# thecasterian/fluca

Hardware: AMD Instinct MI355X
Metric: pressure-Poisson Jacobi-PCG iterations/s, 512^3 cells per GPU (higher is better)
Workload: dtype f64

## Files before the change

### fluca_amd/csrc/fl_knobs.h

```cpp
#pragma once
#include <atomic>

#define FL_PUBLIC_KNOBS(X)                                                                                                                   \
  X(cheb_fuse, 1)                   \
  X(placement, 0)                           \
  X(cg_xbatch, 1)                                           \
  X(cg_xdepth, 8)                 \
  X(cheb_zero3, 1)                  \
  X(mg_prolong, 1)                                                             \
  X(mg_flexible, 1)                                                             \
  X(mg_coarse, 1)                                   \
  X(mg_post_smooth, 0)               \
  X(schur_var_fused, 1)      \
  X(overlap, 1)              \
  X(comm_loopback, 0)           \
  X(comm_trace, 0)                             \
  X(ghost_width, 0)                                       \
  X(placement_verbose, 0)                                                                        \
  X(placement_vmm, 1)                    \
  X(allreduce, 0)

namespace fl {

enum Knob : int {
#define X(n, d) K_##n,
  FL_PUBLIC_KNOBS(X)
#undef X
      K_COUNT
};

int         knob(Knob k);
void        knob_set(Knob k, int v);
int         knob_find(const char *name);
const char *knob_name(int k);

}
```

### fluca_amd/csrc/fl_mg.hip

```cpp
#include <new>

#include "fl_handle.h"
#include "fl_device.h"

namespace fl {

struct Owned {
  int64_t npair_row, npairs;
};
__device__ __forceinline__ Owned owned_of(const GridP &g)
{
  Owned o;
  o.npair_row = (g.nx + 1) / 2;
  o.npairs    = o.npair_row * (int64_t)g.ny * g.nz;
  return o;
}
__device__ __forceinline__ int64_t pair_off(const GridP &g, const Owned &o, int64_t q, bool &two)
{
  const int     ip = (int)(q % o.npair_row);
  const int64_t row = q / o.npair_row;
  const int     j = (int)(row % g.ny), k = (int)(row / g.ny);
  two = 2 * ip + 1 < g.nx;
  return g.off0 + (int64_t)k * g.sxy + (int64_t)j * g.sx + 2 * ip;
}
__device__ __forceinline__ double2 ldp(const double *a, int64_t off, bool two) { return two ? *reinterpret_cast<const double2 *>(a + off) : make_double2(a[off], 0.); }
__device__ __forceinline__ void    stp(double *a, int64_t off, bool two, double2 v)
{
  if (two) *reinterpret_cast<double2 *>(a + off) = v;
  else a[off] = v.x;
}

__global__ void __launch_bounds__(256) k_mg_restrict(GridP gc, GridP gf, int rx, int ry, int rz, const double *__restrict__ wx, const double *__restrict__ wy, const double *__restrict__ wz,
                                                     const double *__restrict__ fine, double *__restrict__ coarse)
{
  const int64_t n = (int64_t)gc.nx * gc.ny * gc.nz;
  for (int64_t q = (int64_t)blockIdx.x * blockDim.x + threadIdx.x; q < n; q += (int64_t)gridDim.x * blockDim.x) {
    const int     I = (int)(q % gc.nx);
    const int64_t t = q / gc.nx;
    const int     J = (int)(t % gc.ny), K = (int)(t / gc.ny);
    double        s = 0.;
    for (int c = 0; c < rz; ++c)
      for (int b = 0; b < ry; ++b) {
        const int     j = J * ry + b, k = K * rz + c;
        const int64_t ro = gf.off0 + (int64_t)k * gf.sxy + (int64_t)j * gf.sx + (int64_t)I * rx;
        const double  wyz = wy[j] * wz[k];
        if (rx == 2) {
          const double2 f = *reinterpret_cast<const double2 *>(fine + ro);
          s += wyz * (wx[2 * I] * f.x + wx[2 * I + 1] * f.y);
        } else s += wyz * wx[I] * fine[ro];
      }
    coarse[gc.off0 + (int64_t)K * gc.sxy + (int64_t)J * gc.sx + I] = s;
  }
}

__global__ void __launch_bounds__(256) k_mg_prolong_add(GridP gf, GridP gc, int rx, int ry, int rz, const double *__restrict__ coarse, double *__restrict__ fine)
{
  const Owned o = owned_of(gf);
  for (int64_t q = (int64_t)blockIdx.x * blockDim.x + threadIdx.x; q < o.npairs; q += (int64_t)gridDim.x * blockDim.x) {
    const int     ip = (int)(q % o.npair_row);
    const int64_t row = q / o.npair_row;
    const int     j = (int)(row % gf.ny), k = (int)(row / gf.ny), i = 2 * ip;
    const bool    two = i + 1 < gf.nx;
    const int64_t fo = gf.off0 + (int64_t)k * gf.sxy + (int64_t)j * gf.sx + i;
    const int64_t co = gc.off0 + (int64_t)(k / rz) * gc.sxy + (int64_t)(j / ry) * gc.sx;
    double2       f = ldp(fine, fo, two);
    f.x += coarse[co + i / rx];
    if (two) f.y += coarse[co + (i + 1) / rx];
    stp(fine, fo, two, f);
  }
}

struct MgLin {
  const int    *pn[3];
  const double *pw[3];
};

__global__ void __launch_bounds__(256) k_mg_prolong_lin_tile(GridP gf, GridP gc, int rx, int ry, int rz, MgLin t, const double *__restrict__ coarse, double *__restrict__ fine, int zc)
{
  const int lane = threadIdx.x & 63, w = __builtin_amdgcn_readfirstlane(threadIdx.x >> 6);
  const int i = ((int)blockIdx.x * 64 + lane) * 2, j = (int)blockIdx.y * 4 + w;
  if (j >= gf.ny || i >= gf.nx) return;
  const int     k0 = (int)blockIdx.z * zc, k1 = min(k0 + zc, gf.nz);
  const bool    two = i + 1 < gf.nx;
  const int     i1 = two ? i + 1 : i;
  const int     I0 = i / rx, I1 = i1 / rx, J = j / ry;
  const int     ox0 = t.pn[0][i], ox1 = t.pn[0][i1];
  const double  wx0 = t.pw[0][i], wx1 = t.pw[0][i1];
  const double  wy = t.pw[1][j];
  const int64_t oy = (int64_t)t.pn[1][j] * gc.sx;
  const double *cj = coarse + gc.off0 + (int64_t)J * gc.sx;
  double       *fj = fine + gf.off0 + (int64_t)j * gf.sx + i;
  for (int k = k0; k < k1; ++k) {
    const int     K = k / rz;
    const double  wz = t.pw[2][k];
    const int64_t oz = (int64_t)t.pn[2][k] * gc.sxy;
    const double *ck = cj + (int64_t)K * gc.sxy;
    double        v0[4], v1[4];
#pragma unroll
    for (int a = 0; a < 4; ++a) {
      const double *line = ck + ((a & 1) ? oy : 0) + ((a & 2) ? oz : 0);
      const double  p0 = line[I0], p1 = line[I1];
      v0[a] = fma(wx0, line[I0 + ox0] - p0, p0);
      v1[a] = fma(wx1, line[I1 + ox1] - p1, p1);
    }
    const double a0 = fma(wy, v0[1] - v0[0], v0[0]), b0 = fma(wy, v0[3] - v0[2], v0[2]);
    const double a1 = fma(wy, v1[1] - v1[0], v1[0]), b1 = fma(wy, v1[3] - v1[2], v1[2]);
    const int64_t fo = (int64_t)k * gf.sxy;
    double2       f = ldp(fj, fo, two);
    f.x += fma(wz, b0 - a0, a0);
    if (two) f.y += fma(wz, b1 - a1, a1);
    stp(fj, fo, two, f);
  }
}

template <int CTRL>
__device__ __forceinline__ double mg_lane_shift(double v)
{
  const int lo = __builtin_amdgcn_update_dpp(__double2loint(v), __double2loint(v), CTRL, 0xf, 0xf, false);
  const int hi = __builtin_amdgcn_update_dpp(__double2hiint(v), __double2hiint(v), CTRL, 0xf, 0xf, false);
  return __hiloint2double(hi, lo);
}
__global__ void __launch_bounds__(256) k_mg_prolong_lin_cc(GridP gf, GridP gc, MgLin t, const double *__restrict__ coarse, double *__restrict__ fine, int kc)
{
  const int lane = threadIdx.x & 63, w = __builtin_amdgcn_readfirstlane(threadIdx.x >> 6);
  const int J = (int)blockIdx.y * 4 + w;
  if (J >= gc.ny) return;
  const int  I = (int)blockIdx.x * 62 - 1 + lane, Ic = min(I, gc.nx);
  const bool act = lane >= 1 && lane <= 62 && I < gc.nx;
  const int  K0 = (int)blockIdx.z * kc, K1 = min(K0 + kc, gc.nz);
  const int  ia = act ? 2 * I : 0;
  const int    ox[2] = {t.pn[0][ia], t.pn[0][ia + 1]};
  const double wx[2] = {t.pw[0][ia], t.pw[0][ia + 1]};
  const int    oy[2] = {t.pn[1][2 * J], t.pn[1][2 * J + 1]};
  const double wy[2] = {t.pw[1][2 * J], t.pw[1][2 * J + 1]};
  const double *cb = coarse + gc.off0 + (int64_t)J * gc.sx + Ic;
  auto plane = [&](int K, double (&X)[3][2]) {
    const double *cp = cb + (int64_t)K * gc.sxy;
#pragma unroll
    for (int jj = 0; jj < 3; ++jj) {
      const double C = cp[(int64_t)(jj - 1) * gc.sx];
      const double L = mg_lane_shift<0x138>(C), R = mg_lane_shift<0x130>(C);
#pragma unroll
      for (int a = 0; a < 2; ++a) {
        const double N = ox[a] < 0 ? L : (ox[a] > 0 ? R : C);
        X[jj][a] = fma(wx[a], N - C, C);
      }
    }
  };
  double Xm[3][2], Xc[3][2], Xp[3][2];
  plane(K0 - 1, Xm);
  plane(K0, Xc);
  for (int K = K0; K < K1; ++K) {
    plane(K + 1, Xp);
#pragma unroll
    for (int c = 0; c < 2; ++c) {
      const int    k = 2 * K + c, oz = t.pn[2][k];
      const double wz = t.pw[2][k];
#pragma unroll
      for (int b = 0; b < 2; ++b) {
        double2 add;
#pragma unroll
        for (int a = 0; a < 2; ++a) {
          const double v0 = Xc[1][a], v1 = oy[b] < 0 ? Xc[0][a] : (oy[b] > 0 ? Xc[2][a] : Xc[1][a]);
          const double z0 = oz < 0 ? Xm[1][a] : (oz > 0 ? Xp[1][a] : Xc[1][a]);
          const double z1 = oz < 0 ? (oy[b] < 0 ? Xm[0][a] : (oy[b] > 0 ? Xm[2][a] : Xm[1][a]))
                                   : (oz > 0 ? (oy[b] < 0 ? Xp[0][a] : (oy[b] > 0 ? Xp[2][a] : Xp[1][a])) : v1);
          const double A = fma(wy[b], v1 - v0, v0), B = fma(wy[b], z1 - z0, z0);
          (a ? add.y : add.x) = fma(wz, B - A, A);
        }
        if (act) {
          double2 *f = reinterpret_cast<double2 *>(fine + gf.off0 + (int64_t)k * gf.sxy + (int64_t)(2 * J + b) * gf.sx + 2 * I);
          double2  v = *f;
          v.x += add.x;
          v.y += add.y;
          *f = v;
        }
      }
    }
#pragma unroll
    for (int jj = 0; jj < 3; ++jj)
#pragma unroll
      for (int a = 0; a < 2; ++a) {
        Xm[jj][a] = Xc[jj][a];
        Xc[jj][a] = Xp[jj][a];
      }
  }
}

__global__ void __launch_bounds__(256) k_mg_dots(GridP g, const double *__restrict__ z, const double *__restrict__ r, double *__restrict__ partial, int stride)
{
  __shared__ double red[5 * 4];
  double            v[5] = {0., 0., 0., 0., 0.};
  const Owned       o = owned_of(g);
  for (int64_t q = (int64_t)blockIdx.x * blockDim.x + threadIdx.x; q < o.npairs; q += (int64_t)gridDim.x * blockDim.x) {
    bool          two;
    const int64_t off = pair_off(g, o, q, two);
    const double2 zv = ldp(z, off, two), rv = ldp(r, off, two);
    v[0] += zv.x + zv.y;
    v[1] += zv.x * zv.x + zv.y * zv.y;
    v[2] += rv.x * zv.x + rv.y * zv.y;
    v[3] += rv.x + rv.y;
    v[4] += rv.x * rv.x + rv.y * rv.y;
  }
  block_sum<5>(v, red);
  if (threadIdx.x == 0)
#pragma unroll
    for (int a = 0; a < 5; ++a) partial[(int64_t)a * stride + blockIdx.x] = v[a];
}

template <int OP>
__global__ void __launch_bounds__(256) k_mg_pw(GridP g, double a, double b, double c, const double *__restrict__ x0, const double *__restrict__ x1, double *__restrict__ y0, double *__restrict__ y1)
{
  const int     lane = threadIdx.x & 63, w = __builtin_amdgcn_readfirstlane(threadIdx.x >> 6), nw = blockDim.x >> 6;
  const int     nseg = (g.nx + 127) / 128;
  const int64_t nitem = (int64_t)nseg * g.ny * g.nz;
  for (int64_t it = (int64_t)blockIdx.x * nw + w; it < nitem; it += (int64_t)gridDim.x * nw) {
    const int seg = (int)(it % nseg), row = (int)(it / nseg);
    const int j = row % g.ny, k = row / g.ny, i = seg * 128 + 2 * lane;
    if (i >= g.nx) continue;
    const bool    two = i + 1 < g.nx;
    const int64_t off = g.off0 + (int64_t)k * g.sxy + (int64_t)j * g.sx + i;
    if (OP == 0) {
      const double2 xv = ldp(x0, off, two), yv = ldp(y0, off, two);
      stp(y0, off, two, make_double2((xv.x - c) + b * yv.x, (xv.y - c) + b * yv.y));
    } else if (OP == 1) {
      const double2 pv = ldp(x0, off, two), qv = ldp(x1, off, two), xv = ldp(y0, off, two), rv = ldp(y1, off, two);
      stp(y0, off, two, make_double2(xv.x + a * pv.x, xv.y + a * pv.y));
      stp(y1, off, two, make_double2(rv.x - a * qv.x, rv.y - a * qv.y));
    } else if (OP == 3) {
      const double2 pv = ldp(x0, off, two), xv = ldp(y0, off, two);
      stp(y0, off, two, make_double2(xv.x + a * pv.x, xv.y + a * pv.y));
    } else if (OP == 4) {
      const double2 zv = ldp(x0, off, two), pv = ldp(y0, off, two), xv = ldp(y1, off, two);
      stp(y1, off, two, make_double2(xv.x + a * pv.x, xv.y + a * pv.y));
      stp(y0, off, two, make_double2((zv.x - c) + b * pv.x, (zv.y - c) + b * pv.y));
    } else if (OP == 5) {
      const double2 qv = ldp(x1, off, two), rv = ldp(y1, off, two);
      stp(y1, off, two, make_double2(rv.x - a * qv.x, rv.y - a * qv.y));
    } else {
      const double2 xv = ldp(x0, off, two);
      stp(y0, off, two, make_double2(xv.x - c, xv.y - c));
    }
  }
}

struct MgScal {
  double alpha, beta, m, rz, rz_old, pq, dp, N;
  int    ns, pnorm, bad_pq, pad_;
};
struct MgSlot {
  double dp, rz, pq;
  int    bad_pq, pad_;
};
template <int STEP, bool FIRST = false>
__global__ void k_mg_scal(MgScal *__restrict__ S, const double *__restrict__ sums, MgSlot *__restrict__ slot_dev)
{
  if (STEP == 0) {
    const double pq = sums[2];
    S->pq     = pq;
    S->bad_pq = !(pq > 0.);
    S->alpha  = pq > 0. ? S->rz / pq : 0.;
  } else if (STEP == 1) {
    const double d0 = sums[0], d1 = sums[1], d2 = sums[2], d3 = sums[3], d4 = sums[4], N = S->N;
    const double m  = S->ns ? d0 / N : 0.;
    const double zz = d1 - N * m * m;
    double       dp = S->pnorm ? sqrt(zz > 0. ? zz : 0.) : sqrt(d4);
    if (isnan(d1)) dp = d1;
    if (!FIRST) S->rz_old = S->rz;
    S->m  = m;
    S->dp = dp;
    S->rz = d2 - m * d3;
    slot_dev->dp     = dp;
    slot_dev->rz     = S->rz;
    slot_dev->pq     = S->pq;
    slot_dev->bad_pq = FIRST ? 0 : S->bad_pq;
  } else if (STEP == 2) {
    S->beta = -S->alpha * (sums[2] - S->m * sums[3]) / S->rz_old;
  } else {
    S->beta = S->rz / S->rz_old;
  }
}

__global__ void k_mg_scal_set(MgScal *dst, MgScal v) { *dst = v; }

constexpr int MG_COARSE_MAX = 4096, MG_COARSE_CPT = MG_COARSE_MAX / 256;
__global__ void __launch_bounds__(256) k_mg_coarse_cg(GridP g, int perbits, int ns, double rtol, double atol, double dtol, int maxit, const double *__restrict__ b, double *__restrict__ x)
{
  constexpr int CPT = MG_COARSE_CPT;
  __shared__ double P[MG_COARSE_MAX];
  __shared__ double red[4 * 4], bc[4];
  const int tid = threadIdx.x, n = g.nx * g.ny * g.nz;
  double    xr[CPT], rr[CPT], di[CPT];
  int       cell_i[CPT], cell_j[CPT], cell_k[CPT];
  auto sum4 = [&](double (&v)[4]) {
    block_sum<4>(v, red);
    if (tid == 0)
#pragma unroll
      for (int a = 0; a < 4; ++a) bc[a] = v[a];
    __syncthreads();
#pragma unroll
    for (int a = 0; a < 4; ++a) v[a] = bc[a];
    __syncthreads();
  };
#pragma unroll
  for (int m = 0; m < CPT; ++m) {
    const int c = tid + 256 * m, cc = min(c, n - 1);
    const int i = cc % g.nx, t = cc / g.nx, j = t % g.ny, k = t / g.ny;
    cell_i[m] = i;
    cell_j[m] = j;
    cell_k[m] = k;
    di[m]     = 1. / (g.sc[0][i] + g.sc[1][j] + g.sc[2][k]);
    xr[m]     = 0.;
    rr[m]     = c < n ? b[pidx(g, i, j, k)] : 0.;
  }
  const double N = (double)n;
  double       beta, betaold = 1., mz, dp, rnorm0, ttol;
  auto pc_sums = [&]() {
    double v[4] = {0., 0., 0., 0.};
#pragma unroll
    for (int m = 0; m < CPT; ++m)
      if (tid + 256 * m < n) {
        const double z = rr[m] * di[m];
        v[0] += z;
        v[1] += z * z;
        v[2] += rr[m] * z;
        v[3] += rr[m];
      }
    sum4(v);
    mz              = ns ? v[0] / N : 0.;
    const double zz = v[1] - N * mz * mz;
    dp              = sqrt(zz > 0. ? zz : 0.);
    if (isnan(v[1])) dp = v[1];
    beta = v[2] - mz * v[3];
  };
  pc_sums();
  rnorm0     = dp;
  ttol       = fmax(rtol * dp, atol);
  auto done = [&](double v) { return isnan(v) || isinf(v) || v <= ttol || v >= dtol * rnorm0; };
  int  it   = 0;
  bool stop = done(dp);
  while (!stop && it < maxit && !(beta < 0.)) {
    const double bb = it == 0 ? 0. : beta / betaold;
#pragma unroll
    for (int m = 0; m < CPT; ++m) {
      const int c = tid + 256 * m;
      if (c < n) P[c] = (rr[m] * di[m] - mz) + (it == 0 ? 0. : bb * P[c]);
    }
    betaold = beta;
    __syncthreads();
    double wv[CPT], v[4] = {0., 0., 0., 0.};
#pragma unroll
    for (int m = 0; m < CPT; ++m) {
      const int c = tid + 256 * m;
      wv[m]       = 0.;
      if (c < n) {
        const int i = cell_i[m], j = cell_j[m], k = cell_k[m];
        const int im = i > 0 ? i - 1 : ((perbits & 1) ? g.nx - 1 : i), ip = i < g.nx - 1 ? i + 1 : ((perbits & 1) ? 0 : i);
        const int jm = j > 0 ? j - 1 : ((perbits & 2) ? g.ny - 1 : j), jp = j < g.ny - 1 ? j + 1 : ((perbits & 2) ? 0 : j);
        const int km = k > 0 ? k - 1 : ((perbits & 4) ? g.nz - 1 : k), kp = k < g.nz - 1 ? k + 1 : ((perbits & 4) ? 0 : k);
        const int row = (k * g.ny + j) * g.nx;
        double    acc = (g.sc[0][i] + g.sc[1][j] + g.sc[2][k]) * P[c];
        acc += g.sl[0][i] * P[row + im] + g.sh[0][i] * P[row + ip];
        acc += g.sl[1][j] * P[(k * g.ny + jm) * g.nx + i] + g.sh[1][j] * P[(k * g.ny + jp) * g.nx + i];
        acc += g.sl[2][k] * P[(km * g.ny + j) * g.nx + i] + g.sh[2][k] * P[(kp * g.ny + j) * g.nx + i];
        wv[m] = acc;
        v[0] += P[c] * acc;
      }
    }
    sum4(v);
    const double dpi = v[0];
    if (!(dpi > 0.)) break;
    const double a = beta / dpi;
#pragma unroll
    for (int m = 0; m < CPT; ++m) {
      const int c = tid + 256 * m;
      if (c < n) {
        xr[m] += a * P[c];
        rr[m] -= a * wv[m];
      }
    }
    pc_sums();
    ++it;
    stop = done(dp);
  }
#pragma unroll
  for (int m = 0; m < CPT; ++m)
    if (tid + 256 * m < n) x[pidx(g, cell_i[m], cell_j[m], cell_k[m])] = xr[m];
}

template <int OP>
__global__ void __launch_bounds__(256) k_mg_pwd(GridP g, const MgScal *__restrict__ S, const double *__restrict__ x0, const double *__restrict__ x1, double *__restrict__ y0, double *__restrict__ y1)
{
  const double  a = S->alpha, b = S->beta, c = S->m;
  const int     lane = threadIdx.x & 63, w = __builtin_amdgcn_readfirstlane(threadIdx.x >> 6), nw = blockDim.x >> 6;
  const int     nseg = (g.nx + 127) / 128;
  const int64_t nitem = (int64_t)nseg * g.ny * g.nz;
  for (int64_t it = (int64_t)blockIdx.x * nw + w; it < nitem; it += (int64_t)gridDim.x * nw) {
    const int seg = (int)(it % nseg), row = (int)(it / nseg);
    const int j = row % g.ny, k = row / g.ny, i = seg * 128 + 2 * lane;
    if (i >= g.nx) continue;
    const bool    two = i + 1 < g.nx;
    const int64_t off = g.off0 + (int64_t)k * g.sxy + (int64_t)j * g.sx + i;
    if (OP == 2) {
      const double2 xv = ldp(x0, off, two);
      stp(y0, off, two, make_double2(xv.x - c, xv.y - c));
    } else if (OP == 4) {
      const double2 zv = ldp(x0, off, two), pv = ldp(y0, off, two), xv = ldp(y1, off, two);
      stp(y1, off, two, make_double2(xv.x + a * pv.x, xv.y + a * pv.y));
      stp(y0, off, two, make_double2((zv.x - c) + b * pv.x, (zv.y - c) + b * pv.y));
    } else {
      const double2 qv = ldp(x1, off, two), rv = ldp(y1, off, two);
      stp(y1, off, two, make_double2(rv.x - a * qv.x, rv.y - a * qv.y));
    }
  }
}

}

using namespace fl;

struct MgLevel {
  fl_poisson *h = nullptr;
  int         r[3] = {1, 1, 1};
  double     *w[3] = {nullptr, nullptr, nullptr};
  int        *pn[3] = {nullptr, nullptr, nullptr};
  double     *pw[3] = {nullptr, nullptr, nullptr};
  double     *x = nullptr, *b = nullptr;
};

struct fl_mg {
  std::vector<MgLevel> lv;
  int                  requested = 0;
  MgScal              *scal = nullptr;
  MgSlot              *slot_dev = nullptr;
  MgSlot              *slot_host = nullptr;
  hipEvent_t           ev_slot[2] = {nullptr, nullptr};
};

void fl_mg_destroy(fl_poisson *h);

static inline int fl_mg_prolong_mode() { return knob(K_mg_prolong); }

static inline int fl_mg_flexible_mode() { return knob(K_mg_flexible); }

static inline int fl_mg_coarse_mode() { return knob(K_mg_coarse); }

namespace {

constexpr int MG_BLOCKS = 4096;

int nblk(int64_t n) { return (int)std::max<int64_t>(1, std::min<int64_t>((n + 255) / 256, MG_BLOCKS)); }
int nblk_pairs(const GridP &g) { return nblk((int64_t)((g.nx + 1) / 2) * g.ny * g.nz); }

int dots(fl_poisson *h, const double *z, const double *r, double out[5])
{
  const int nb = nblk_pairs(h->g);
  hipLaunchKernelGGL(k_mg_dots, dim3(nb), dim3(256), 0, h->stream, h->g, z, r, h->partial, h->partial_stride);
  launch_reduce(h->stream, h->partial, nb, h->partial_stride, 5, h->sums);
  if (h->multi) FL_CHK(h->comm.allreduce(h->stream, h->sums, NSLOT));
  FL_HIP(hipMemcpyAsync(out, h->sums, sizeof(double) * 5, hipMemcpyDeviceToHost, h->stream));
  FL_HIP(hipStreamSynchronize(h->stream));
  return 0;
}

int alloc_cells(fl_poisson *h, double **p) { return fl_dev_alloc(h, (void **)p, sizeof(double) * (size_t)h->ncell, true); }

int mg_build_levels(fl_poisson *h, fl_mg *mg, int max_levels);

int mg_build(fl_poisson *h, int max_levels)
{
  h->mg = new (std::nothrow) fl_mg;
  if (!h->mg) return FL_ERR_MEM;
  const int rc = mg_build_levels(h, h->mg, max_levels);
  if (rc != 0) fl_mg_destroy(h);
  return rc;
}

int mg_build_levels(fl_poisson *h, fl_mg *mg, int max_levels)
{
  MgLevel L0;
  L0.h = h;
  mg->lv.push_back(L0);
  for (int l = 0; max_levels <= 0 || l + 1 < max_levels; ++l) {
    fl_poisson *hf = mg->lv[l].h;
    int         r[3];
    bool        any = false;
    for (int d = 0; d < 3; ++d) {
      const int64_t n = hf->ax[d].n, m = hf->dec.ranks[d];
      r[d] = (n % (2 * m) == 0 && n / m >= 8 && hf->dec.lo[d] % 2 == 0 && hf->dec.len[d] % 2 == 0) ? 2 : 1;
    }
    if (hf->multi) {
      FL_HIP(hipStreamSynchronize(hf->stream));
      double ok[NSLOT] = {0., 0., 0., 0., 0., 0., 0., 0.};
      for (int d = 0; d < 3; ++d) ok[d] = r[d] == 2 ? 0. : 1.;
      FL_HIP(hipMemcpy(hf->sums, ok, sizeof(ok), hipMemcpyHostToDevice));
      FL_CHK(hf->comm.allreduce(hf->stream, hf->sums, NSLOT));
      FL_HIP(hipMemcpyAsync(ok, hf->sums, sizeof(ok), hipMemcpyDeviceToHost, hf->stream));
      FL_HIP(hipStreamSynchronize(hf->stream));
      for (int d = 0; d < 3; ++d)
        if (ok[d] != 0.) r[d] = 1;
    }
    for (int d = 0; d < 3; ++d) any |= r[d] == 2;
    if (!any) break;
    std::vector<double> xf[3];
    fl_grid             cg;
    for (int d = 0; d < 3; ++d) {
      const int64_t nc = hf->ax[d].n / r[d];
      xf[d].resize((size_t)nc + 1);
      for (int64_t i = 0; i <= nc; ++i) xf[d][(size_t)i] = hf->ax[d].xf[(size_t)(i * r[d])];
      cg.n[d]  = nc;
      cg.xf[d] = xf[d].data();
      cg.xc[d] = nullptr;
    }
    fl_poisson *hc = nullptr;
    fl_decomp   cd = hf->dec;
    for (int d = 0; d < 3; ++d) {
      cd.lo[d] /= r[d];
      cd.len[d] /= r[d];
    }
    if (fl_poisson_create(&cg, h->bc, h->kappa, h->multi ? &cd : nullptr, h->device, &hc) != 0) break;
    if (h->multi) hc->comm.borrow(h->comm);
    MgLevel Lc;
    Lc.h = hc;
    mg->lv.push_back(Lc);
    FL_CHK(fl_poisson_set_stream(hc, (void *)h->stream));
    for (int d = 0; d < 3; ++d) {
      mg->lv[l].r[d] = r[d];
      std::vector<double> w((size_t)hf->dec.len[d]);
      for (int64_t il = 0; il < hf->dec.len[d]; ++il) {
        const int64_t i = hf->dec.lo[d] + il, I = i / r[d];
        w[(size_t)il]   = (hf->ax[d].xf[(size_t)i + 1] - hf->ax[d].xf[(size_t)i]) / (xf[d][(size_t)I + 1] - xf[d][(size_t)I]);
      }
      FL_HIP(hipMalloc((void **)&mg->lv[l].w[d], sizeof(double) * w.size()));
      FL_HIP(hipMemcpy(mg->lv[l].w[d], w.data(), sizeof(double) * w.size(), hipMemcpyHostToDevice));
      std::vector<int>    pn((size_t)hf->dec.len[d], 0);
      std::vector<double> pw((size_t)hf->dec.len[d], 0.);
      if (r[d] == 2) {
        const int64_t nc = hf->ax[d].n / 2;
        const double  L = xf[d][(size_t)nc] - xf[d][0];
        auto          Xc = [&](int64_t I) {
          if (I < 0) return 0.5 * (xf[d][(size_t)(I + nc)] + xf[d][(size_t)(I + nc) + 1]) - L;
          if (I >= nc) return 0.5 * (xf[d][(size_t)(I - nc)] + xf[d][(size_t)(I - nc) + 1]) + L;
          return 0.5 * (xf[d][(size_t)I] + xf[d][(size_t)I + 1]);
        };
        for (int64_t il = 0; il < hf->dec.len[d]; ++il) {
          const int64_t i = hf->dec.lo[d] + il, I = i / 2, In = (i % 2) ? I + 1 : I - 1;
          if (!hf->ax[d].periodic && (In < 0 || In >= nc)) continue;
          const double xc = 0.5 * (hf->ax[d].xf[(size_t)i] + hf->ax[d].xf[(size_t)i + 1]);
          pn[(size_t)il] = (i % 2) ? 1 : -1;
          pw[(size_t)il] = (xc - Xc(I)) / (Xc(In) - Xc(I));
        }
      }
      FL_HIP(hipMalloc((void **)&mg->lv[l].pn[d], sizeof(int) * std::max<size_t>(pn.size(), 1)));
      FL_HIP(hipMalloc((void **)&mg->lv[l].pw[d], sizeof(double) * std::max<size_t>(pw.size(), 1)));
      FL_HIP(hipMemcpy(mg->lv[l].pn[d], pn.data(), sizeof(int) * pn.size(), hipMemcpyHostToDevice));
      FL_HIP(hipMemcpy(mg->lv[l].pw[d], pw.data(), sizeof(double) * pw.size(), hipMemcpyHostToDevice));
    }
  }
  for (size_t l = 0; l < mg->lv.size(); ++l) {
    MgLevel    &L = mg->lv[l];
    fl_poisson *hl = L.h;
    for (double **v : {&hl->r, &hl->P0, &hl->q, &hl->xp}) FL_CHK(fl_ensure_vec(hl, v));
    if (l + 1 == mg->lv.size()) {
      FL_CHK(alloc_cells(hl, &L.x));
      FL_CHK(alloc_cells(hl, &L.b));
    }
    FL_CHK(fl_ensure_partials(hl, MG_BLOCKS));
  }
  for (double **v : {&h->w0, &h->w1, &h->w2}) FL_CHK(fl_ensure_vec(h, v));
  FL_HIP(hipMalloc((void **)&mg->scal, sizeof(MgScal)));
  FL_HIP(hipMalloc((void **)&mg->slot_dev, 2 * sizeof(MgSlot)));
  FL_HIP(hipHostMalloc((void **)&mg->slot_host, 2 * sizeof(MgSlot)));
  for (hipEvent_t &e : mg->ev_slot) FL_HIP(hipEventCreateWithFlags(&e, hipEventDisableTiming));
  return 0;
}

int vcycle(fl_mg *mg, size_t l, const fl_ksp_opts *o, bool *sums = nullptr, const double *subq = nullptr)
{
  const bool want = sums && *sums;
  if (sums) *sums = false;
  MgLevel    &L = mg->lv[l];
  fl_poisson *h = L.h;
  if (l + 1 == mg->lv.size()) {
    fl_ksp_stats st;
    fl_ksp_opts  so;
    fl_ksp_opts_default(&so);
    so.remove_nullspace = o->remove_nullspace;
    so.type  = FL_KSP_CG;
    so.pc    = FL_PC_JACOBI;
    so.rtol  = 1e-2;
    so.maxit = 200;
    if (subq) hipLaunchKernelGGL(k_mg_pwd<5>, dim3(nblk_pairs(h->g)), dim3(256), 0, h->stream, h->g, (const MgScal *)mg->scal, (const double *)nullptr, subq, (double *)nullptr, h->r);
    if (!h->multi && h->ncell <= MG_COARSE_MAX && fl_mg_coarse_mode() != 0) {
      const int per = (h->ax[0].periodic ? 1 : 0) | (h->ax[1].periodic ? 2 : 0) | (h->ax[2].periodic ? 4 : 0);
      hipLaunchKernelGGL(k_mg_coarse_cg, dim3(1), dim3(256), 0, h->stream, h->g, per, so.remove_nullspace, so.rtol, so.atol, so.dtol, so.maxit, (const double *)h->r, h->xp);
      return 0;
    }
    launch_unpad_copy(h->stream, h->g, h->r, L.b, nullptr);
    if (l == 0) {
      FL_CHK(fl_ensure_vec(h, &h->cd1));
      FL_HIP(hipMemcpyAsync(h->cd1, h->r, sizeof(double) * h->padlen, hipMemcpyDeviceToDevice, h->stream));
    }
    FL_CHK(fl_poisson_solve(h, L.b, L.x, &so, &st));
    if (l == 0) FL_HIP(hipMemcpyAsync(h->r, h->cd1, sizeof(double) * h->padlen, hipMemcpyDeviceToDevice, h->stream));
    launch_pad_copy(h->stream, h->g, L.x, h->xp);
    return 0;
  }
  const int nu = o->mg_smooth_its > 0 ? o->mg_smooth_its : 3;
  MgLevel  &C  = mg->lv[l + 1];
  FL_CHK(fl_cheb_smooth_padded(h, nu, true, true, nullptr, subq, subq ? &mg->scal->alpha : nullptr));
  int fused = 1;
  if (L.r[0] == 2 && L.r[1] == 2 && L.r[2] == 2) {
    fused = fl_residual_restrict_padded(h, h->xp, h->r, L.w[0], L.w[1], L.w[2], C.h, C.h->r);
    if (fused < 0) return fused;
  }
  if (fused != 0) {
    FL_CHK(fl_residual_padded(h, h->xp, h->r, h->q));
    hipLaunchKernelGGL(k_mg_restrict, dim3(nblk(C.h->ncell)), dim3(256), 0, h->stream, C.h->g, h->g, L.r[0], L.r[1], L.r[2], L.w[0], L.w[1], L.w[2], h->q, C.h->r);
  }
  FL_CHK(vcycle(mg, l + 1, o));
  if (fl_mg_prolong_mode() == 1) {
    FL_CHK(fl_fill_ghosts_full(C.h, C.h->xp));
    MgLin t;
    for (int d = 0; d < 3; ++d) {
      t.pn[d] = L.pn[d];
      t.pw[d] = L.pw[d];
    }
    if (L.r[0] == 2 && L.r[1] == 2 && L.r[2] == 2) {
      const int  kc = 4;
      const GridP &gcs = C.h->g;
      hipLaunchKernelGGL(k_mg_prolong_lin_cc, dim3((gcs.nx + 61) / 62, (gcs.ny + 3) / 4, (gcs.nz + kc - 1) / kc), dim3(256), 0, h->stream, h->g, gcs, t, (const double *)C.h->xp, h->xp, kc);
    } else {
      const int  zc = 8;
      const dim3 grid((h->g.nx + 127) / 128, (h->g.ny + 3) / 4, (h->g.nz + zc - 1) / zc);
      hipLaunchKernelGGL(k_mg_prolong_lin_tile, grid, dim3(256), 0, h->stream, h->g, C.h->g, L.r[0], L.r[1], L.r[2], t, (const double *)C.h->xp, h->xp, zc);
    }
  } else hipLaunchKernelGGL(k_mg_prolong_add, dim3(nblk_pairs(h->g)), dim3(256), 0, h->stream, h->g, C.h->g, L.r[0], L.r[1], L.r[2], C.h->xp, h->xp);
  bool got = want;
  const int nu_post = knob(K_mg_post_smooth) > 0 ? knob(K_mg_post_smooth) : nu;
  FL_CHK(fl_cheb_smooth_padded(h, nu_post, true, false, &got));
  if (sums) *sums = got;
  return 0;
}

}

void fl_mg_destroy(fl_poisson *h)
{
  fl_mg *mg = h->mg;
  if (!mg) return;
  for (size_t l = 0; l < mg->lv.size(); ++l) {
    MgLevel &L = mg->lv[l];
    for (double *p : {L.x, L.b, L.w[0], L.w[1], L.w[2], L.pw[0], L.pw[1], L.pw[2]})
      if (p) (void)hipFree(p);
    for (int *p : L.pn)
      if (p) (void)hipFree(p);
    if (l > 0 && L.h) fl_poisson_destroy(L.h);
  }
  if (mg->scal) (void)hipFree(mg->scal);
  if (mg->slot_dev) (void)hipFree(mg->slot_dev);
  if (mg->slot_host) (void)hipHostFree(mg->slot_host);
  for (hipEvent_t e : mg->ev_slot)
    if (e) (void)hipEventDestroy(e);
  delete mg;
  h->mg = nullptr;
}

void fl_mg_set_stream(fl_poisson *h)
{
  if (!h->mg) return;
  for (size_t l = 1; l < h->mg->lv.size(); ++l) (void)fl_poisson_set_stream(h->mg->lv[l].h, (void *)h->stream);
}

int fl_solve_cg_mg(fl_poisson *h, const double *b, double *x, const fl_ksp_opts *o, fl_ksp_stats *st)
{
  if (h->multi && h->comm.kind == Comm::NONE) return FL_ERR_ARG_WRONGSTATE;
  if (o->norm_type != FL_NORM_PRECONDITIONED && o->norm_type != FL_NORM_UNPRECONDITIONED) return FL_ERR_SUP;
  if (h->mg && h->mg->requested != o->mg_levels) fl_mg_destroy(h);
  if (!h->mg) {
    FL_CHK(mg_build(h, o->mg_levels));
    h->mg->requested = o->mg_levels;
  }
  for (double **v : {&h->r, &h->P0, &h->q, &h->xp, &h->w0, &h->w1, &h->w2}) FL_CHK(fl_ensure_vec(h, v));
  fl_mg       *mg = h->mg;
  const GridP &g = h->g;
  const bool   ns = o->remove_nullspace != 0;
  const bool   pnorm = o->norm_type == FL_NORM_PRECONDITIONED;
  const double N = (double)h->ax[0].n * (double)h->ax[1].n * (double)h->ax[2].n;
  const int    nb = nblk_pairs(g);
  hipStream_t  s = h->stream;
  struct Events {
    hipEvent_t a = nullptr, b = nullptr;
    ~Events()
    {
      if (a) (void)hipEventDestroy(a);
      if (b) (void)hipEventDestroy(b);
    }
  } ev;
  FL_HIP(hipEventCreate(&ev.a));
  FL_HIP(hipEventCreate(&ev.b));
  hipEvent_t e0 = ev.a, e1 = ev.b;
  FL_HIP(hipEventRecord(e0, s));
  double *X = h->w0, *P = h->w1, *Q = h->w2;
  double  d[5], rz = 0., dp = 0., pq = 0.;
  int     bad_pq = 0;
  std::vector<double> hist;
  MgScal *S = mg->scal;
  {
    MgScal init;
    std::memset(&init, 0, sizeof(init));
    init.N      = N;
    init.ns     = ns ? 1 : 0;
    init.pnorm  = pnorm ? 1 : 0;
    init.rz_old = 1.;
    hipLaunchKernelGGL(k_mg_scal_set, dim3(1), dim3(1), 0, s, S, init);
  }
  auto dots_dev = [&](const double *z, const double *r) -> int {
    hipLaunchKernelGGL(k_mg_dots, dim3(nb), dim3(256), 0, s, g, z, r, h->partial, h->partial_stride);
    launch_reduce(s, h->partial, nb, h->partial_stride, 5, h->sums);
    if (h->multi) FL_CHK(h->comm.allreduce(s, h->sums, NSLOT));
    return 0;
  };
  const double *subq = nullptr;
  auto cycle_and_sums = [&](int it, bool first) -> int {
    bool got = true;
    FL_CHK(vcycle(mg, 0, o, &got, subq));
    if (!got) FL_CHK(dots_dev(h->xp, h->r));
    const int a = it & 1;
    if (first) hipLaunchKernelGGL((k_mg_scal<1, true>), dim3(1), dim3(1), 0, s, S, (const double *)h->sums, mg->slot_dev + a);
    else hipLaunchKernelGGL((k_mg_scal<1, false>), dim3(1), dim3(1), 0, s, S, (const double *)h->sums, mg->slot_dev + a);
    FL_HIP(hipMemcpyAsync(mg->slot_host + a, mg->slot_dev + a, sizeof(MgSlot), hipMemcpyDeviceToHost, s));
    FL_HIP(hipEventRecord(mg->ev_slot[a], s));
    return 0;
  };
  auto look = [&](int it) -> int {
    const int a = it & 1;
    FL_HIP(hipEventSynchronize(mg->ev_slot[a]));
    const MgSlot &L = mg->slot_host[a];
    dp     = L.dp;
    rz     = L.rz;
    pq     = L.pq;
    bad_pq = L.bad_pq;
    return 0;
  };
  launch_pad_copy(s, g, b, h->r);
  FL_CHK(fl_zero_vec(h, X));
  FL_CHK(cycle_and_sums(0, true));
  hipLaunchKernelGGL(k_mg_pwd<2>, dim3(nb), dim3(256), 0, s, g, (const MgScal *)S, (const double *)h->xp, (const double *)nullptr, P, (double *)nullptr);
  FL_CHK(look(0));
  const double rnorm0 = dp, ttol = std::max(o->rtol * dp, o->atol);
  hist.push_back(dp);
  int  it = 0, reason = 0;
  auto converged = [&](double v) {
    if (std::isnan(v) || std::isinf(v)) return (int)FL_DIVERGED_NANORINF;
    if (v <= ttol) return v < o->atol ? (int)FL_CONVERGED_ATOL : (int)FL_CONVERGED_RTOL;
    if (v >= o->dtol * rnorm0) return (int)FL_DIVERGED_DTOL;
    return 0;
  };
  reason = converged(dp);
  if (!reason && o->maxit <= 0) reason = FL_DIVERGED_ITS;
  const bool flexible = fl_mg_flexible_mode() != 0;
  while (!reason) {
    FL_CHK(fl_apply_padded_dot(h, P, Q, nullptr));
    hipLaunchKernelGGL((k_mg_scal<0>), dim3(1), dim3(1), 0, s, S, (const double *)h->sums, (MgSlot *)nullptr);
    subq = Q;
    FL_CHK(cycle_and_sums(it + 1, false));
    subq = nullptr;
    if (flexible) {
      FL_CHK(dots_dev(h->xp, Q));
      hipLaunchKernelGGL((k_mg_scal<2>), dim3(1), dim3(1), 0, s, S, (const double *)h->sums, (MgSlot *)nullptr);
    } else hipLaunchKernelGGL((k_mg_scal<3>), dim3(1), dim3(1), 0, s, S, (const double *)h->sums, (MgSlot *)nullptr);
    hipLaunchKernelGGL(k_mg_pwd<4>, dim3(nb), dim3(256), 0, s, g, (const MgScal *)S, (const double *)h->xp, (const double *)nullptr, P, X);
    FL_CHK(look(it + 1));
    if (bad_pq) {
      reason = std::isnan(pq) ? FL_DIVERGED_NANORINF : FL_DIVERGED_INDEFINITE_MAT;
      break;
    }
    ++it;
    hist.push_back(dp);
    reason = converged(dp);
    if (!reason && it >= o->maxit) reason = FL_DIVERGED_ITS;
    if (!reason && !(rz > 0.)) reason = std::isnan(rz) ? FL_DIVERGED_NANORINF : FL_DIVERGED_INDEFINITE_PC;
  }
  double *shift = nullptr;
  if (ns) {
    FL_CHK(dots(h, X, X, d));
    const double mx = d[0] / N;
    FL_HIP(hipMemcpyAsync(h->sums, &mx, sizeof(double), hipMemcpyHostToDevice, s));
    FL_HIP(hipStreamSynchronize(s));
    shift = h->sums;
  }
  launch_unpad_copy(s, g, X, x, shift);
  FL_HIP(hipEventRecord(e1, s));
  FL_HIP(hipStreamSynchronize(s));
  float ms = 0.f;
  FL_HIP(hipEventElapsedTime(&ms, e0, e1));
  st->iters   = it;
  st->reason  = reason;
  if (reason == FL_DIVERGED_NANORINF || reason == FL_DIVERGED_DTOL || !std::isfinite(dp)) {
    for (MgLevel &L : mg->lv) L.h->poisoned = true;
  } else {
    for (MgLevel &L : mg->lv) L.h->poisoned = false;
  }
  st->rnorm0  = rnorm0;
  st->rnorm   = dp;
  st->seconds = ms * 1e-3;
  if (o->history && o->nhistory > 0) {
    const int n = std::min<int>(o->nhistory, (int)hist.size());
    std::memcpy(o->history, hist.data(), sizeof(double) * n);
  }
  return 0;
}
```

Baseline: 716.1.

## Fuse MG-PCG direction update, x update, and next operator apply into one kernel

```diff
diff --git a/fluca_amd/csrc/fl_knobs.h b/fluca_amd/csrc/fl_knobs.h
--- a/fluca_amd/csrc/fl_knobs.h
+++ b/fluca_amd/csrc/fl_knobs.h
@@ -11,7 +11,8 @@
   X(mg_flexible, 1)                                                             \
   X(mg_coarse, 1)                                   \
   X(mg_post_smooth, 0)               \
-  X(schur_var_fused, 1)      \
+  X(mg_fused_dir, 1)        \
+  X(schur_var_fused, 1)     \
   X(overlap, 1)              \
   X(comm_loopback, 0)           \
   X(comm_trace, 0)                             \
diff --git a/fluca_amd/csrc/fl_mg.hip b/fluca_amd/csrc/fl_mg.hip
--- a/fluca_amd/csrc/fl_mg.hip
+++ b/fluca_amd/csrc/fl_mg.hip
@@ -2,6 +2,7 @@
 
 #include "fl_handle.h"
 #include "fl_device.h"
+#include "fl_stencil.h"
 
 namespace fl {
 
@@ -415,6 +416,159 @@
   }
 }
 
+template <int RY, int NW>
+__global__ void __launch_bounds__(64 * NW, 2) k_mg_dir(GridP g, const MgScal *__restrict__ S, const double *__restrict__ z, const double *__restrict__ pold, double *__restrict__ pnew, double *__restrict__ x, double *__restrict__ q,
+                                                       double *__restrict__ partial, int stride, int nchunk, int zc, int tiles_x, int tiles, int remap)
+{
+  using T           = TileA<RY, NW>;
+  constexpr int TX = T::TX, TY = T::TY, LX = T::LX, LY = T::LY;
+  __shared__ __attribute__((aligned(16))) double lds[3][LY][LX];
+  __shared__ double                              red[4 * NW];
+  const double alpha = S->alpha, beta = S->beta, msh = S->m;
+
+  const int b     = remap ? xcd_remap(blockIdx.x, gridDim.x) : blockIdx.x;
+  const int chunk = b / tiles, tile = b % tiles;
+  const int i0 = (tile % tiles_x) * TX, j0 = (tile / tiles_x) * TY;
+  const int k0 = chunk * zc, k1 = min(k0 + zc, g.nz);
+  const int tid = threadIdx.x, lane = tid & 63;
+  const int w  = __builtin_amdgcn_readfirstlane(tid >> 6);
+  const int i  = i0 + 2 * lane;
+  const int jb = j0 + w * RY;
+
+  const bool   own0 = i < g.nx, own1 = i + 1 < g.nx;
+  const int    il  = min(i, g.nx & ~1);
+  const int    ic0 = min(i, g.nx), ic1 = min(i + 1, g.nx);
+  const double xl0 = g.sl[0][ic0], xc0 = g.sc[0][ic0], xh0 = g.sh[0][ic0];
+  const double xl1 = g.sl[0][ic1], xc1 = g.sc[0][ic1], xh1 = g.sh[0][ic1];
+  int64_t rob[RY];
+  bool    rown[RY];
+  double  yl[RY], yc[RY], yh[RY];
+#pragma unroll
+  for (int m = 0; m < RY; ++m) {
+    const int j = jb + m, jc = min(j, g.ny);
+    rown[m]     = j < g.ny;
+    rob[m]      = g.off0 + (int64_t)jc * g.sx + il;
+    yl[m]       = g.sl[1][jc];
+    yc[m]       = g.sc[1][jc];
+    yh[m]       = g.sh[1][jc];
+  }
+  constexpr int HB0 = NW > 4 ? 256 : 0;
+  const int     tb  = tid - HB0;
+  const int     hAi = i0 + (tid & 127), hAj = j0 + (tid < 128 ? -1 : TY);
+  const bool    hAok = tid < 256 && hAi < g.nx && hAj <= g.ny;
+  const int     hBi = i0 + ((tb & 1) ? TX : -1), hBj = j0 + (tb >> 1);
+  const bool    hBok = tb >= 0 && tb < 2 * TY && hBj < g.ny && hBi <= g.nx;
+  const int64_t tbase = g.off0 + (int64_t)j0 * g.sx + i0;
+  const int     hAo   = hAok ? (hAj - j0) * g.sx + (hAi - i0) : 0;
+  const int     hBo   = hBok ? (hBj - j0) * g.sx + (hBi - i0) : 0;
+  const int     hAr = hAok ? (tid < 128 ? 0 : TY + 1) : 0, hAc = hAok ? (tid & 127) + 2 : 0;
+  const int     hBr = hBok ? (tb >> 1) + 1 : 0, hBc = hBok ? ((tb & 1) ? TX + 2 : 1) : 0;
+
+  double acc[4] = {0., 0., 0., 0.};
+  double zlc = 0., zcc = 0., zhc = 0.;
+  struct Raw {
+    double2 z[RY], p[RY], x[RY];
+    double  zA, zB, pA, pB;
+    double  zl, zc, zh;
+  };
+  auto load = [&](int kn_, Raw &R) {
+    const int     kn = min(kn_, k1);
+    const int64_t pl = (int64_t)kn * g.sxy, px = (int64_t)min(max(kn_, k0), k1 - 1) * g.sxy;
+#pragma unroll
+    for (int m = 0; m < RY; ++m) {
+      R.z[m] = ld2<1>(z + rob[m] + pl);
+      R.p[m] = ld2<1>(pold + rob[m] + pl);
+      R.x[m] = ld2<1>(x + rob[m] + px);
+    }
+    R.zA = z[tbase + pl + hAo];
+    R.zB = z[tbase + pl + hBo];
+    R.pA = pold[tbase + pl + hAo];
+    R.pB = pold[tbase + pl + hBo];
+    R.zl = g.sl[2][kn];
+    R.zc = g.sc[2][kn];
+    R.zh = g.sh[2][kn];
+  };
+  auto step = [&](int kk, Raw &C, Raw &N) {
+    load(kk + 1, N);
+    const double nzl = C.zl, nzc = C.zc, nzh = C.zh;
+    const int    buf = (kk + 3) % 3;
+    const int    kc  = kk - 1;
+    double2 sv[RY];
+#pragma unroll
+    for (int m = 0; m < RY; ++m) {
+      sv[m].x = (C.z[m].x - msh) + beta * C.p[m].x;
+      sv[m].y = (C.z[m].y - msh) + beta * C.p[m].y;
+    }
+    if (kc >= k0) {
+      const int     bc = (kc + 3) % 3, bp = (kc + 2) % 3;
+      const int64_t pc = (int64_t)kc * g.sxy;
+      const int     lc = 2 * lane + 2;
+#pragma unroll
+      for (int m = 0; m < RY; ++m) {
+        const int     lr = w * RY + m + 1;
+        const double2 cen   = *reinterpret_cast<const double2 *>(&lds[bc][lr][lc]);
+        const double2 south = *reinterpret_cast<const double2 *>(&lds[bc][lr - 1][lc]);
+        const double2 north = *reinterpret_cast<const double2 *>(&lds[bc][lr + 1][lc]);
+        const double2 below = *reinterpret_cast<const double2 *>(&lds[bp][lr][lc]);
+        const double  west = lds[bc][lr][lc - 1], east = lds[bc][lr][lc + 2];
+        const double  dyc = yc[m] + zcc;
+        double2       y;
+        y.x = st7(xc0 + dyc, cen.x, xl0, west, xh0, cen.y, yl[m], south.x, yh[m], north.x, zlc, below.x, zhc, sv[m].x);
+        y.y = st7(xc1 + dyc, cen.y, xl1, cen.x, xh1, east, yl[m], south.y, yh[m], north.y, zlc, below.y, zhc, sv[m].y);
+        const bool o0 = rown[m] && own0, o1 = rown[m] && own1;
+        if (o1) st2<1>(q + rob[m] + pc, y);
+        else if (o0) q[rob[m] + pc] = y.x;
+        acc[0] += (o0 ? y.x : 0.) + (o1 ? y.y : 0.);
+        acc[2] += (o0 ? cen.x * y.x : 0.) + (o1 ? cen.y * y.y : 0.);
+        acc[3] += (o0 ? y.x * y.x : 0.) + (o1 ? y.y * y.y : 0.);
+      }
+    }
+    const bool    mine = kk >= k0 && kk < k1;
+    const int64_t pk   = (int64_t)kk * g.sxy;
+#pragma unroll
+    for (int m = 0; m < RY; ++m) {
+      *reinterpret_cast<double2 *>(&lds[buf][w * RY + m + 1][2 * lane + 2]) = sv[m];
+      if (mine) {
+        const bool    o0 = rown[m] && own0, o1 = rown[m] && own1;
+        const double2 xn = make_double2(C.x[m].x + alpha * C.p[m].x, C.x[m].y + alpha * C.p[m].y);
+        if (o1) {
+          st2<1>(x + rob[m] + pk, xn);
+          st2<1>(pnew + rob[m] + pk, sv[m]);
+        } else if (o0) {
+          x[rob[m] + pk]    = xn.x;
+          pnew[rob[m] + pk] = sv[m].x;
+        }
+      }
+    }
+    lds[buf][hAr][hAc] = (C.zA - msh) + beta * C.pA;
+    lds[buf][hBr][hBc] = (C.zB - msh) + beta * C.pB;
+    __syncthreads();
+    zlc = nzl;
+    zcc = nzc;
+    zhc = nzh;
+  };
+  {
+    Raw A, B;
+    load(k0 - 1, A);
+    for (int kk = k0 - 1; kk <= k1; kk += 2) {
+      step(kk, A, B);
+      if (kk + 1 <= k1) step(kk + 1, B, A);
+    }
+  }
+#pragma unroll
+  for (int a = 0; a < 4; ++a) {
+    acc[a] = wave_sum(acc[a]);
+    if (lane == 0) red[a * NW + w] = acc[a];
+  }
+  __syncthreads();
+  if (tid < 4) {
+    double t = 0.;
+#pragma unroll
+    for (int n = 0; n < NW; ++n) t += red[tid * NW + n];
+    partial[(int64_t)tid * stride + blockIdx.x] = t;
+  }
+}
+
 }
 
 using namespace fl;
@@ -435,6 +589,7 @@
   MgSlot              *slot_dev = nullptr;
   MgSlot              *slot_host = nullptr;
   hipEvent_t           ev_slot[2] = {nullptr, nullptr};
+  double              *dir2 = nullptr;
 };
 
 void fl_mg_destroy(fl_poisson *h);
@@ -643,6 +798,28 @@
   return 0;
 }
 
+template <int RY, int NW>
+void mg_dir_t(fl_poisson *h, const PlanA &p, const MgScal *S, const double *z, const double *pold, double *pnew, double *x, double *q)
+{
+  hipLaunchKernelGGL((k_mg_dir<RY, NW>), dim3(p.nblocks), dim3(64 * NW), 0, h->stream, h->g, S, z, pold, pnew, x, q, h->partial, h->partial_stride, p.nchunk, p.zc, p.tiles_x, p.tiles_x * p.tiles_y, p.remap);
+}
+
+int mg_dir(fl_poisson *h, fl_mg *mg, const double *p, double *pnew, double *x, double *q)
+{
+  const bool ghosts = fl_any_ghost_exchange(h);
+  if (ghosts) FL_CHK(fl_fill_ghosts(h, h->xp));
+  const PlanA pa = plan_cg_A(h->g, 0, 0);
+  FL_CHK(fl_ensure_partials(h, pa.nblocks));
+  switch (pa.ry * 10 + pa.nw) {
+  case 28: mg_dir_t<2, 8>(h, pa, mg->scal, h->xp, p, pnew, x, q); break;
+  case 24: mg_dir_t<2, 4>(h, pa, mg->scal, h->xp, p, pnew, x, q); break;
+  default: mg_dir_t<1, 4>(h, pa, mg->scal, h->xp, p, pnew, x, q); break;
+  }
+  launch_reduce(h->stream, h->partial, pa.nblocks, h->partial_stride, 4, h->sums);
+  if (ghosts) FL_CHK(fl_fill_ghosts(h, pnew));
+  return 0;
+}
+
 }
 
 void fl_mg_destroy(fl_poisson *h)
@@ -658,6 +835,7 @@
     if (l > 0 && L.h) fl_poisson_destroy(L.h);
   }
   if (mg->scal) (void)hipFree(mg->scal);
+  if (mg->dir2) (void)hipFree(mg->dir2);
   if (mg->slot_dev) (void)hipFree(mg->slot_dev);
   if (mg->slot_host) (void)hipHostFree(mg->slot_host);
   for (hipEvent_t e : mg->ev_slot)
@@ -702,6 +880,18 @@
   hipEvent_t e0 = ev.a, e1 = ev.b;
   FL_HIP(hipEventRecord(e0, s));
   double *X = h->w0, *P = h->w1, *Q = h->w2;
+  const bool fused_dir = knob(K_mg_fused_dir) != 0 && !h->multi;
+  double    *P2 = nullptr;
+  if (fused_dir) {
+    if (mg->lv.size() == 1) {
+      if (!mg->dir2) FL_CHK(fl_dev_alloc(h, (void **)&mg->dir2, sizeof(double) * h->padlen, true));
+      P2 = mg->dir2;
+    } else {
+      FL_CHK(fl_ensure_vec(h, &h->P1));
+      if (h->poisoned) FL_CHK(fl_zero_vec(h, h->P1));
+      P2 = h->P1;
+    }
+  }
   double  d[5], rz = 0., dp = 0., pq = 0.;
   int     bad_pq = 0;
   std::vector<double> hist;
@@ -760,8 +950,9 @@
   reason = converged(dp);
   if (!reason && o->maxit <= 0) reason = FL_DIVERGED_ITS;
   const bool flexible = fl_mg_flexible_mode() != 0;
+  bool have_q = false;
   while (!reason) {
-    FL_CHK(fl_apply_padded_dot(h, P, Q, nullptr));
+    if (!have_q) FL_CHK(fl_apply_padded_dot(h, P, Q, nullptr));
     hipLaunchKernelGGL((k_mg_scal<0>), dim3(1), dim3(1), 0, s, S, (const double *)h->sums, (MgSlot *)nullptr);
     subq = Q;
     FL_CHK(cycle_and_sums(it + 1, false));
@@ -770,7 +961,11 @@
       FL_CHK(dots_dev(h->xp, Q));
       hipLaunchKernelGGL((k_mg_scal<2>), dim3(1), dim3(1), 0, s, S, (const double *)h->sums, (MgSlot *)nullptr);
     } else hipLaunchKernelGGL((k_mg_scal<3>), dim3(1), dim3(1), 0, s, S, (const double *)h->sums, (MgSlot *)nullptr);
-    hipLaunchKernelGGL(k_mg_pwd<4>, dim3(nb), dim3(256), 0, s, g, (const MgScal *)S, (const double *)h->xp, (const double *)nullptr, P, X);
+    if (fused_dir) {
+      FL_CHK(mg_dir(h, mg, P, P2, X, Q));
+      std::swap(P, P2);
+      have_q = true;
+    } else hipLaunchKernelGGL(k_mg_pwd<4>, dim3(nb), dim3(256), 0, s, g, (const MgScal *)S, (const double *)h->xp, (const double *)nullptr, P, X);
     FL_CHK(look(it + 1));
     if (bad_pq) {
       reason = std::isnan(pq) ? FL_DIVERGED_NANORINF : FL_DIVERGED_INDEFINITE_MAT;
```

Result: no change. 715.0, median of 3 (-0.2%).
